# aantropov/Sailor

Measured on NVIDIA B200. Metric: Mrays/s, higher is better.
Workload: dtype f32

## Files before the change

### sailor_b200/csrc/backend.cu

```cuda
#include "backend.h"
#include "../../include/sailor_pt.h"
#include <chrono>
#include <stdio.h>
#include <array>
#include <mutex>
#include <unordered_map>
#include <thread>
#include <condition_variable>
#include <atomic>
#include <vector>

namespace spt
{
	bool Ctx::Fail(const char* what, int code)
	{
		if (ok)
		{
			ok = false;
			char buf[512];
#if !defined(SPT_EMU)
			snprintf(buf, sizeof(buf), "%s -> %s (%d)", what, cudaGetErrorString((cudaError_t)code), code);
#else
			snprintf(buf, sizeof(buf), "%s -> %d", what, code);
#endif
			error = buf;
		}
		return false;
	}

#if !defined(SPT_EMU)
	namespace
	{
		std::mutex g_pinnedPoolMutex;
		std::vector<uint32_t*> g_pinnedPool;
	}
	int Ctx::Init()
	{
		int count = 0;
		if (cudaGetDeviceCount(&count) != cudaSuccess || count <= 0)
		{
			cudaGetLastError();
			ok = false;
			error = "no CUDA device: the sailor_b200 product library has no CPU path";
			return SAILOR_PT_ERR_NO_DEVICE;
		}
		if (cudaStreamCreateWithFlags(&stream, cudaStreamNonBlocking) != cudaSuccess ||
			cudaEventCreate(&evA) != cudaSuccess || cudaEventCreate(&evB) != cudaSuccess)
		{
			Fail("cudaStreamCreate/cudaEventCreate", (int)cudaGetLastError());
			return SAILOR_PT_ERR_CUDA;
		}
		ok = true;
		return SAILOR_PT_OK;
	}
	void Ctx::Destroy()
	{
		if (pinned)
		{
			std::lock_guard<std::mutex> lock(g_pinnedPoolMutex);
			if (g_pinnedPool.size() < 64) g_pinnedPool.push_back(pinned); else cudaFreeHost(pinned);
			pinned = nullptr;
		}
		if (evA) cudaEventDestroy(evA);
		if (evB) cudaEventDestroy(evB);
		for (int i = 0; i < kMarkers; i++) { if (ev[i]) cudaEventDestroy(ev[i]); ev[i] = nullptr; }
		if (stream) cudaStreamDestroy(stream);
		evA = evB = nullptr; stream = nullptr;
	}
	void Ctx::Sync() { if (ok) SPT_CUDA_CHECK(*this, cudaStreamSynchronize(stream)); }
	void Ctx::TimerStart() { if (ok) SPT_CUDA_CHECK(*this, cudaEventRecord(evA, stream)); }
	double Ctx::TimerStop()
	{
		if (!ok) return 0.0;
		SPT_CUDA_CHECK(*this, cudaEventRecord(evB, stream));
		SPT_CUDA_CHECK(*this, cudaEventSynchronize(evB));
		float ms = 0.0f;
		if (ok) SPT_CUDA_CHECK(*this, cudaEventElapsedTime(&ms, evA, evB));
		return (double)ms * 1e-3;
	}

	void Ctx::Mark(int i)
	{
		if (!ok) return;
		if (!ev[i]) SPT_CUDA_CHECK(*this, cudaEventCreate(&ev[i]));
		if (ok) SPT_CUDA_CHECK(*this, cudaEventRecord(ev[i], stream));
	}
	void Ctx::WaitMark(int i) { if (ok) SPT_CUDA_CHECK(*this, cudaEventSynchronize(ev[i])); }
	uint32_t* Ctx::Pinned()
	{
		if (!pinned && ok)
		{
			{
				std::lock_guard<std::mutex> lock(g_pinnedPoolMutex);
				if (!g_pinnedPool.empty()) { pinned = g_pinnedPool.back(); g_pinnedPool.pop_back(); }
			}
			if (!pinned) { void* p = nullptr; SPT_CUDA_CHECK(*this, cudaHostAlloc(&p, 256 * sizeof(uint32_t), cudaHostAllocPortable)); pinned = (uint32_t*)p; }
		}
		return pinned;
	}
	void Ctx::ReadAsync(uint32_t* pinnedDst, const void* src, size_t bytes)
	{
		d2hBytes += bytes;
		if (ok) SPT_CUDA_CHECK(*this, cudaMemcpyAsync(pinnedDst, src, bytes, cudaMemcpyDeviceToHost, stream));
	}
	double Ctx::Between(int i, int j)
	{
		float ms = 0.0f;
		if (ok) SPT_CUDA_CHECK(*this, cudaEventElapsedTime(&ms, ev[i], ev[j]));
		return (double)ms * 1e-3;
	}

	namespace
	{
		std::mutex g_allocMutex;
		std::unordered_map<void*, cudaStream_t> g_allocStream;
		uint64_t g_poolReady = 0;

		void EnsurePool()
		{
			int dev = 0; cudaMemPool_t pool = nullptr;
			if (cudaGetDevice(&dev) != cudaSuccess) { cudaGetLastError(); return; }
			if (dev < 64 && (g_poolReady >> dev & 1u)) return;
			if (cudaDeviceGetDefaultMemPool(&pool, dev) == cudaSuccess)
			{
				uint64_t threshold = UINT64_MAX;
				cudaMemPoolSetAttribute(pool, cudaMemPoolAttrReleaseThreshold, &threshold);
			}
			cudaGetLastError();
			if (dev < 64) g_poolReady |= 1ull << dev;
		}
	}

	void* DevAllocBytes(Ctx& ctx, size_t bytes)
	{
		void* p = nullptr;
		if (!ctx.ok) return nullptr;
		std::lock_guard<std::mutex> lock(g_allocMutex);
		EnsurePool();
		SPT_CUDA_CHECK(ctx, cudaMallocAsync(&p, bytes, ctx.stream));
		if (!ctx.ok) return nullptr;
		g_allocStream[p] = ctx.stream;
		return p;
	}
	int DevCurrent() { int d = 0; if (cudaGetDevice(&d) != cudaSuccess) { cudaGetLastError(); d = 0; } return d; }
	int DevCount() { int n = 0; if (cudaGetDeviceCount(&n) != cudaSuccess) { cudaGetLastError(); n = 0; } return n; }
	bool DevSetCurrent(int device) { if (cudaSetDevice(device) != cudaSuccess) { cudaGetLastError(); return false; } return true; }
	void DevCopyPeer(Ctx& ctx, void* dst, int dstDevice, const void* src, int srcDevice, size_t bytes)
	{
		if (!ctx.ok || !bytes) return;
		if (dstDevice == srcDevice) SPT_CUDA_CHECK(ctx, cudaMemcpyAsync(dst, src, bytes, cudaMemcpyDeviceToDevice, ctx.stream));
// ... 249 lines not shown
			__syncthreads();
			if (warp == 0)
			{
				uint32_t w = lane < kScanThreads / 32 ? warpSums[lane] : 0;
#pragma unroll
				for (int o = 1; o < 32; o <<= 1) { const uint32_t t = __shfl_up_sync(0xffffffffu, w, o); if (lane >= o) w += t; }
				if (lane < kScanThreads / 32) warpSums[lane] = w;
			}
			__syncthreads();
			total = warpSums[kScanThreads / 32 - 1];
			const uint32_t base = warp ? warpSums[warp - 1] : 0;
			__syncthreads();
			return base + incl - v;
		}

		__global__ void __launch_bounds__(kScanThreads) k_scan_reduce(const uint32_t* __restrict__ in, uint32_t n, uint32_t* __restrict__ tileSums)
		{
			const uint32_t base = blockIdx.x * kScanTile;
			uint32_t s = 0;
#pragma unroll
			for (uint32_t k = 0; k < kScanItems; k++) { const uint32_t i = base + k * kScanThreads + threadIdx.x; if (i < n) s += in[i]; }
			uint32_t total;
			BlockExclusiveScan(s, total);
			if (threadIdx.x == 0) tileSums[blockIdx.x] = total;
		}

		__global__ void __launch_bounds__(kScanThreads) k_scan_tiles(uint32_t* tileSums, uint32_t numTiles)
		{
			uint32_t carry = 0;
			for (uint32_t base = 0; base < numTiles; base += kScanThreads)
			{
				const uint32_t i = base + threadIdx.x;
				const uint32_t v = i < numTiles ? tileSums[i] : 0;
				uint32_t total;
				const uint32_t ex = BlockExclusiveScan(v, total);
				if (i < numTiles) tileSums[i] = carry + ex;
				carry += total;
			}
			if (threadIdx.x == 0) tileSums[numTiles] = carry;
		}

		__global__ void __launch_bounds__(kScanThreads) k_scan_apply(const uint32_t* __restrict__ in, uint32_t* __restrict__ out, uint32_t n, const uint32_t* __restrict__ tileOffsets, uint32_t numTiles)
		{
			const uint32_t base = blockIdx.x * kScanTile + threadIdx.x * kScanItems;
			uint32_t v[kScanItems];
			uint32_t s = 0;
#pragma unroll
			for (uint32_t k = 0; k < kScanItems; k++) { v[k] = (base + k) < n ? in[base + k] : 0; s += v[k]; }
			uint32_t total;
			uint32_t run = tileOffsets[blockIdx.x] + BlockExclusiveScan(s, total);
#pragma unroll
			for (uint32_t k = 0; k < kScanItems; k++) { if ((base + k) < n) out[base + k] = run; run += v[k]; }
			if (blockIdx.x == 0 && threadIdx.x == 0) out[n] = tileOffsets[numTiles];
		}
	}

	void ExclusiveScanU32(Ctx& ctx, const uint32_t* in, uint32_t* out, uint32_t n, DevBuf<uint32_t>& scratch)
	{
		if (!ctx.ok) return;
		if (n == 0) { DevMemset(ctx, out, 0, sizeof(uint32_t)); return; }
		const uint32_t numTiles = (n + kScanTile - 1) / kScanTile;
		scratch.Ensure(ctx, numTiles + 1);
		if (!ctx.ok) return;
		k_scan_reduce<<<numTiles, kScanThreads, 0, ctx.stream>>>(in, n, scratch.p);
		k_scan_tiles<<<1, kScanThreads, 0, ctx.stream>>>(scratch.p, numTiles);
		k_scan_apply<<<numTiles, kScanThreads, 0, ctx.stream>>>(in, out, n, scratch.p, numTiles);
		ctx.kernelLaunches += 3;
		SPT_CUDA_CHECK(ctx, cudaGetLastError());
	}

#else
	static std::chrono::steady_clock::time_point g_t0, g_marks[64];
	static double NowS() { return std::chrono::duration<double>(std::chrono::steady_clock::now().time_since_epoch()).count(); }
	void SpanTimer::Begin(Ctx&) { t0 = NowS(); }
	void SpanTimer::End(Ctx&) { acc += NowS() - t0; used += 2; }
	double SpanTimer::Collect(Ctx&) { const double s = acc; acc = 0.0; used = 0; return s; }
	void SpanTimer::Destroy() {}
	void Ctx::Mark(int i) { g_marks[i] = std::chrono::steady_clock::now(); }
	void Ctx::WaitMark(int) {}
	uint32_t* Ctx::Pinned() { if (!pinned) pinned = (uint32_t*)calloc(256, sizeof(uint32_t)); return pinned; }
	void Ctx::ReadAsync(uint32_t* pinnedDst, const void* src, size_t bytes) { d2hBytes += bytes; memcpy(pinnedDst, src, bytes); }
	double Ctx::Between(int i, int j) { return std::chrono::duration<double>(g_marks[j] - g_marks[i]).count(); }
	int Ctx::Init() { ok = true; return SAILOR_PT_OK; }
	void Ctx::Destroy() { free(pinned); pinned = nullptr; }
	void Ctx::Sync() {}
	void Ctx::TimerStart() { g_t0 = std::chrono::steady_clock::now(); }
	double Ctx::TimerStop() { return std::chrono::duration<double>(std::chrono::steady_clock::now() - g_t0).count(); }
	void* DevAllocBytes(Ctx&, size_t bytes) { return malloc(bytes ? bytes : 1); }
	void DevFreeBytes(void* p) { free(p); }
	size_t DevMemAvailable() { return (size_t)4 << 30; }
	int DevCurrent() { return 0; }
	int DevCount() { return 1; }
	bool DevSetCurrent(int device) { return device == 0; }
	void DevCopyPeer(Ctx&, void* dst, int, const void* src, int, size_t bytes) { memcpy(dst, src, bytes); }
	void TrimDevicePool() {}
	void* DevAllocPlain(Ctx&, size_t bytes) { return malloc(bytes ? bytes : 1); }
	void DevFreePlain(void* p) { free(p); }
	void DevUpload(Ctx& ctx, void* dst, const void* src, size_t bytes) { ctx.h2dBytes += bytes; memcpy(dst, src, bytes); }
	void DevDownload(Ctx& ctx, void* dst, const void* src, size_t bytes) { ctx.d2hBytes += bytes; memcpy(dst, src, bytes); }
	int HostPin(void* p, size_t bytes) { return (p && bytes) ? 0 : -1; }
	int HostUnpin(void* p) { return p ? 0 : -1; }
	void DevMemset(Ctx&, void* dst, int byte, size_t bytes) { memset(dst, byte, bytes); }
	void DevCopy(Ctx&, void* dst, const void* src, size_t bytes) { memcpy(dst, src, bytes); }
	void ExclusiveScanU32(Ctx& ctx, const uint32_t* in, uint32_t* out, uint32_t n, DevBuf<uint32_t>&)
	{
		uint32_t s = 0;
		for (uint32_t i = 0; i < n; i++) { out[i] = s; s += in[i]; }
		out[n] = s;
		ctx.kernelLaunches += 3;
	}
#endif
}
```

### sailor_b200/csrc/backend.h

```cpp
#pragma once
#include "hd.h"
#include <stddef.h>
#include <string>
#include <vector>
#include <string.h>
#include <stdlib.h>

#if !defined(SPT_EMU)
#include <cuda_runtime.h>
#if defined(__CUDACC__)
#include <cooperative_groups.h>
#include <cooperative_groups/scan.h>
#include <cooperative_groups/reduce.h>
#endif
#endif

namespace spt
{
	struct Ctx
	{
#if !defined(SPT_EMU)
		cudaStream_t stream = nullptr;
		cudaEvent_t evA = nullptr, evB = nullptr;
		static constexpr int kMarkers = 64;
		cudaEvent_t ev[kMarkers] = {};
#endif
		uint32_t kernelLaunches = 0;
		uint64_t h2dBytes = 0, d2hBytes = 0;
		static constexpr int kMarkCall0 = 60, kMarkCall1 = 61;
		std::string error;
		bool ok = true;

		int Init();
		void Destroy();
		void Sync();
		bool Fail(const char* what, int code);
		void TimerStart();
		double TimerStop();
		void Mark(int i);
		double Between(int i, int j);
		void WaitMark(int i);
		uint32_t* pinned = nullptr;
		uint32_t* Pinned();
		void ReadAsync(uint32_t* pinnedDst, const void* src, size_t bytes);
	};

#if !defined(SPT_EMU)
#define SPT_CUDA_CHECK(ctx, call) do { cudaError_t e_ = (call); if (e_ != cudaSuccess) { (ctx).Fail(#call, (int)e_); } } while (0)
#endif

	void* DevAllocBytes(Ctx& ctx, size_t bytes);
	int DevCurrent();
	int DevCount();
	bool DevSetCurrent(int device);
	void DevCopyPeer(Ctx& ctx, void* dst, int dstDevice, const void* src, int srcDevice, size_t bytes);
	void TrimDevicePool();
	void* DevAllocPlain(Ctx& ctx, size_t bytes);
	void DevFreePlain(void* p);
	size_t DevMemAvailable();
	void DevFreeBytes(void* p);
	void DevUpload(Ctx& ctx, void* dst, const void* src, size_t bytes);
	void DevDownload(Ctx& ctx, void* dst, const void* src, size_t bytes);
	void DevMemset(Ctx& ctx, void* dst, int byte, size_t bytes);
	int HostPin(void* p, size_t bytes);
	int HostUnpin(void* p);
	void DevCopy(Ctx& ctx, void* dst, const void* src, size_t bytes);

	template<class T>
	struct DevBuf
	{
		T* p = nullptr;
		size_t n = 0;
		DevBuf() = default;
		DevBuf(const DevBuf&) = delete;
		DevBuf& operator=(const DevBuf&) = delete;
		~DevBuf() { Free(); }
		void Free() { if (p) DevFreeBytes(p); p = nullptr; n = 0; }
		void Alloc(Ctx& ctx, size_t count) { Free(); if (count) { p = (T*)DevAllocBytes(ctx, count * sizeof(T)); n = p ? count : 0; } }
		void Ensure(Ctx& ctx, size_t count) { if (count > n) Alloc(ctx, count); }
		void Upload(Ctx& ctx, const T* src, size_t count) { Ensure(ctx, count); if (count) DevUpload(ctx, p, src, count * sizeof(T)); }
		void Upload(Ctx& ctx, const std::vector<T>& v) { Upload(ctx, v.data(), v.size()); }
		void Download(Ctx& ctx, T* dst, size_t count) const { if (count) DevDownload(ctx, dst, p, count * sizeof(T)); }
		void Zero(Ctx& ctx) { if (n) DevMemset(ctx, p, 0, n * sizeof(T)); }
		void Zero(Ctx& ctx, size_t count) { if (count) DevMemset(ctx, p, 0, count * sizeof(T)); }
	};

	struct PlainBuf
	{
		unsigned char* p = nullptr; size_t n = 0;
		void Ensure(Ctx& ctx, size_t bytes)
		{
			if (bytes <= n) return;
			if (p) { ctx.Sync(); DevFreePlain(p); p = nullptr; n = 0; }
			p = (unsigned char*)DevAllocPlain(ctx, bytes); n = p ? bytes : 0;
		}
	};

#if !defined(SPT_EMU)
	__device__ __forceinline__ void atomic_min_u32(uint32_t* p, uint32_t v) { atomicMin(p, v); }
	__device__ __forceinline__ void atomic_max_u32(uint32_t* p, uint32_t v) { atomicMax(p, v); }
	__device__ __forceinline__ uint32_t atomic_add_u32(uint32_t* p, uint32_t v) { return atomicAdd(p, v); }
	__device__ __forceinline__ unsigned long long atomic_add_u64(unsigned long long* p, unsigned long long v) { return atomicAdd(p, v); }
#define SPT_KERNEL_BODY __device__ __forceinline__
#if defined(__CUDACC__)
	__device__ __forceinline__ uint32_t atomic_inc_u32_agg(uint32_t* p)
	{
		const uint32_t mask = __activemask(), lane = threadIdx.x & 31u;
		const int leader = __ffs(mask) - 1;
		uint32_t base = 0;
		if ((int)lane == leader) base = atomicAdd(p, (uint32_t)__popc(mask));
		base = __shfl_sync(mask, base, leader);
		return base + (uint32_t)__popc(mask & ((1u << lane) - 1u));
	}
	__device__ __forceinline__ uint32_t atomic_add_u32_agg(uint32_t* p, uint32_t v)
	{
		namespace cg = cooperative_groups;
		const cg::coalesced_group g = cg::coalesced_threads();
		const uint32_t excl = cg::exclusive_scan(g, v);
		const uint32_t last = g.size() - 1u;
		uint32_t base = 0;
		if (g.thread_rank() == last) base = atomicAdd(p, excl + v);
		base = g.shfl(base, last);
		return base + excl;
	}
	__device__ __forceinline__ void atomic_add_u64_agg(unsigned long long* p, unsigned long long v)
	{
		namespace cg = cooperative_groups;
// ... 92 lines not shown
```

### sailor_b200/csrc/integrator.cuh

```cuda
#pragma once
#include "pipeline.cuh"
#include "textures.cuh"
#include "lighting.cuh"
#include "blue_noise_table.h"

namespace spt
{
	struct alignas(16) PrimaryHitRec { uint32_t pixel, sample, pad0, pad1; float t, u, v; uint32_t tri; };
	static_assert(sizeof(PrimaryHitRec) == 32, "PrimaryHitRec layout");

	struct RenderStats { uint64_t rays, primarySamples, fanOutSamples, replayedRays; double secondsTraverse, secondsShade, secondsStage[4]; uint32_t traverseLaunches, batches; };

	constexpr uint32_t kNone = 0xFFFFFFFFu;
#ifndef SPT_FAN_OUT_MIN
#define SPT_FAN_OUT_MIN 8
#endif
	constexpr uint32_t kFanOutMinSamples = SPT_FAN_OUT_MIN;

	enum : uint32_t
	{
		kNfOpposite = 1u, kNfThick = 2u, kNfAlpha = 4u, kNfFirst = 8u, kNfAmbientOn = 16u,
		kNfDone = 32u,
		kNfTail = 64u,
		kNfLevel0 = 128u,
	};

	struct alignas(16) NodeRec
	{
		V3 rayO; float envIor;
		V3 rayD; uint32_t pad0;
		float t, u, v; uint32_t tri;
		float inAcc; uint32_t pNum; uint64_t rngKey;
		uint32_t bounces, flags, auxBase; float alpha;
		uint32_t parent, parentAux, nA, nS;
		V3 emissive; uint32_t child;
		V3 result; uint32_t pad1;
	};
	SPT_HD uint32_t PackNum(uint32_t samples, uint32_t ambient) { return (samples & 0xFFFFu) | (ambient << 16); }
	static_assert(sizeof(NodeRec) == 128, "NodeRec layout");

	enum : uint32_t
	{
		kRkInactive = 0, kRkLight = 1, kRkHemi = 2, kRkSample = 3, kRkOwn = 4, kRkMask = 7u,
		kRsTransRay = 16u,
		kRsHit = 64u,
		kRsSky2 = 256u,
		kRsSkipped = 512u,
	};

	struct alignas(16) RayAux
	{
		float a0, a1, a2, a3;
		float b0, b1, b2;
		uint32_t tag;
	};
	static_assert(sizeof(RayAux) == 32, "RayAux layout");

	struct alignas(16) SkyState
	{
		V3 att; uint32_t targetAux;
		V3 prev; uint32_t ignore;
		V3 start; float ior;
		V3 dir; uint32_t jAndMax;
	};
	static_assert(sizeof(SkyState) == 64, "SkyState layout");

	struct ShadeCtx;
	struct LevelInfo { uint32_t recBegin, recEnd, rayCount, auxBase; };

	struct BatchCounters
	{
		uint32_t recAlloc;
		uint32_t auxAlloc;
		uint32_t overflow;
		uint32_t skyCount[2];
		uint32_t zero;
		uint32_t fanEntries;
		uint32_t slowCount;
		uint32_t fanThreads[2];
		unsigned long long rays;
		unsigned long long fanSamples;
		LevelInfo level[66];
	};

	struct IntegratorArgs
	{
		const V4* shade; const V4* centroid; const MaterialGpu* materials; TextureSet tex; const V4* lights; uint32_t numLights;
		const uint16_t* blueNoise;
		CameraGpu cam; uint32_t rowBegin, rowEnd, msBegin, msEnd, msaa;
		uint32_t maxBounces, numSamples, numAmbientSamples; V3 ambient; uint64_t seed;
		const PrimaryHitRec* hitQueue; uint32_t queueBegin, queueCount;
		NodeRec* recs; uint32_t recCap;
		RayAux* aux; uint32_t auxCap; uint32_t hasSky;
		RayRec* rays; Hit* hits; uint32_t rayCap;
		uint8_t* status; SlowRec* slow;
		SkyState* sky[2]; RayRec* skyRays; Hit* skyHits; uint32_t skyCap;
		ShadeCtx* fan; uint32_t fanCap; uint32_t* fanSlots[2];
		BatchCounters* c;
		float* sampleBuf;
	};

	SPT_HD uint64_t Mix64(uint64_t z)
	{
		z = (z ^ (z >> 30)) * 0xBF58476D1CE4E5B9ULL; z = (z ^ (z >> 27)) * 0x94D049BB133111EBULL; return z ^ (z >> 31);
	}
	SPT_HD uint64_t PrimaryRngKey(uint64_t seed, uint32_t pixel, uint32_t msaa, uint32_t sample)
	{
		return Mix64(seed * 0x9E3779B97F4A7C15ULL + ((uint64_t)pixel * msaa + sample) + 0x632BE59BD9B4E019ULL);
	}
	SPT_HD uint64_t ChildRngKey(uint64_t key, uint32_t slot) { return Mix64(key + 0xD1B54A32D192ED03ULL * (uint64_t)(slot + 1u)); }
	struct Rng
	{
		uint64_t key; uint32_t counter;
		SPT_KERNEL_BODY uint32_t U32()
		{
			const uint64_t h = Mix64(key + 0x9E3779B97F4A7C15ULL * (uint64_t)(++counter));
			const uint32_t b0 = (uint32_t)(h & 0xFFFF) % 255u, b1 = (uint32_t)((h >> 16) & 0xFFFF) % 255u;
			const uint32_t b2 = (uint32_t)((h >> 32) & 0xFFFF) % 255u, b3 = (uint32_t)((h >> 48) & 0xFFFF) % 255u;
			return (b3 << 24) | (b2 << 16) | (b1 << 8) | b0;
		}
		SPT_KERNEL_BODY float Float01() { return (float)U32() / 4294967296.0f * (1.0f - 0.0f) + 0.0f; }
		SPT_KERNEL_BODY uint32_t Seed681() { return U32() % 681u; }
	};

	SPT_KERNEL_BODY uint32_t MaterialOfTri(const IntegratorArgs& a, uint32_t tri) { return f2u(ld4(a.centroid + tri).w); }

	SPT_KERNEL_BODY V3 HitNormalOf(const IntegratorArgs& a, uint32_t tri, float u, float v)
	{
		const V4* S = a.shade + (size_t)tri * 9;
		const V4 n0 = ld4(S), n1 = ld4(S + 1), n2 = ld4(S + 2);
		const float w = 1.0f - u - v;
		return w * v3(n0.x, n0.y, n0.z) + u * v3(n1.x, n1.y, n1.z) + v * v3(n2.x, n2.y, n2.z);
	}

	SPT_KERNEL_BODY void WriteRay(RayRec* q, uint32_t i, V3 o, V3 d, uint32_t ignore, bool active, bool anyHit = false)
	{
		RayRec r; r.ox = o.x; r.oy = o.y; r.oz = o.z; r.ignoreTri = ignore; r.dx = d.x; r.dy = d.y; r.dz = d.z; r.tmax = active ? (anyHit ? -kFltMax : kFltMax) : -1.0f;
		q[i] = r;
	}

	SPT_KERNEL_BODY void WriteAux(const IntegratorArgs& a, uint32_t g, float a0, float a1, float a2, float a3, float b0, uint32_t tag, uint32_t owner)
	{
		RayAux x; x.a0 = a0; x.a1 = a1; x.a2 = a2; x.a3 = a3; x.b0 = b0; x.b1 = u2f(owner); x.b2 = 0.0f; x.tag = tag;
		a.aux[g] = x;
	}

	SPT_KERNEL_BODY uint32_t AllocRecord(const IntegratorArgs& a)
	{
		const uint32_t i = atomic_inc_u32_agg(&a.c->recAlloc);
		if (i >= a.recCap) { a.c->overflow = 1u; return kNone; }
		return i;
	}

	SPT_KERNEL_BODY bool SkyAdvance(const IntegratorArgs& a, SkyState& s, const Hit& hit, V3& result)
	{
		if (hit.tri == kNoHit) { result = s.att; return false; }
		const MaterialGpu& m = a.materials[MaterialOfTri(a, hit.tri)];
		const V3 hn = HitNormalOf(a, hit.tri, hit.u, hit.v);
		const bool hitOpp = dot(s.dir, hn) < 0.0f;
		if (!(m.transmission > 0.0f && m.thickness > 0.0f)) { result = v3(0.0f); return false; }
		const V3 hp = s.start + s.dir * hit.t;
		const float distance = length(hp - s.prev);
		s.prev = hp;
		const V3 wn = hitOpp ? hn : -hn;
// ... 598 lines not shown
							if (x.tag & kRsSkipped) continue;
							V3 value = v3(x.a0, x.a1, x.a2);
							if (!hitSomething[j])
							{
								value = glm_clamp(value * a.ambient, 0.0f, 10.0f);
								amb2 = amb2 + value; avgPdf += x.a3; indirect = indirect + value;
							}
							else if (x.tag & kRsHit)
							{
								indirect = indirect + value;
								if (x.tag & kRsSky2) { amb2 = amb2 + value * v3(x.b0, x.b1, x.b2); avgPdf += x.a3; }
							}
							else if (bouncesLeft)
								indirect = indirect + glm_clamp(value * v3(0.0f), 0.0f, 10.0f);
							cnt += 1.0f;
						}
						g += (nS - i0 < kGatherBlock) ? nS - i0 : kGatherBlock;
					}
					amb2 = amb2 / cnt; avgPdf = avgPdf / cnt;
					const V3 ambient = amb1 + amb2;
					if (ambient.x + ambient.y + ambient.z > 0.0f)
					{
						res = res + (amb1 * PowerHeuristic((int32_t)nA, pdfHemisphere, (int32_t)cnt, avgPdf) +
							amb2 * PowerHeuristic((int32_t)cnt, avgPdf, (int32_t)nA, pdfHemisphere));
					}
					if (cnt > 0.0f) res = res + (indirect / cnt);
				}
				res = res + rec->emissive;
				if ((rec->bounces & 0xFFFFu) > 0 && (flags & kNfAlpha))
				{
					const float al = rec->alpha;
					const V3 cr = rec->child != kNone ? a.recs[rec->child].result : v3(0.0f);
					res = res * al + cr * (1.0f - al);
				}
			}
			rec->result = res;
			if (flags & kNfLevel0)
			{
				const uint32_t pixel = rec->parent, sample = rec->parentAux;
				const uint32_t x = pixel % a.cam.width, y = pixel / a.cam.width;
				const size_t idx = ((size_t)(y - a.rowBegin) * a.cam.width + x) * (a.msEnd - a.msBegin) + (sample - a.msBegin);
				a.sampleBuf[idx * 3] = res.x; a.sampleBuf[idx * 3 + 1] = res.y; a.sampleBuf[idx * 3 + 2] = res.z;
			}
			else if (rec->parentAux != kNone)
			{
				RayAux* px = a.aux + rec->parentAux;
				const V3 value = glm_clamp(v3(px->a0, px->a1, px->a2) * res, 0.0f, 10.0f);
				px->a0 = value.x; px->a1 = value.y; px->a2 = value.z;
			}
		}
	};

	struct BeginBatchKernel
	{
		BatchCounters* c; uint32_t count;
		SPT_KERNEL_BODY void operator()(uint32_t) const
		{
			c->recAlloc = count; c->auxAlloc = 0; c->overflow = 0; c->skyCount[0] = c->skyCount[1] = 0; c->zero = 0; c->fanEntries = 0; c->fanThreads[0] = c->fanThreads[1] = 0; c->slowCount = 0; c->rays = 0; c->fanSamples = 0;
			c->level[0].recBegin = 0; c->level[0].recEnd = count; c->level[0].rayCount = 0; c->level[0].auxBase = 0;
		}
	};
	struct NextLevelKernel
	{
		BatchCounters* c; uint32_t level; uint32_t recCap;
		SPT_KERNEL_BODY void operator()(uint32_t) const
		{
			const LevelInfo cur = c->level[level];
			LevelInfo nx; nx.recBegin = cur.recEnd; nx.recEnd = c->recAlloc < recCap ? c->recAlloc : recCap; nx.rayCount = 0; nx.auxBase = cur.auxBase + cur.rayCount;
			c->level[level + 1] = nx;
			c->auxAlloc = nx.auxBase;
			c->rays += cur.rayCount;
			c->fanEntries = 0; c->fanThreads[0] = c->fanThreads[1] = 0; c->slowCount = 0;
		}
	};
	struct OverflowGuardKernel
	{
		BatchCounters* c; uint32_t level;
		SPT_KERNEL_BODY void operator()(uint32_t) const
		{
			if (!c->overflow) return;
			c->level[level].rayCount = 0; c->slowCount = 0; c->skyCount[0] = c->skyCount[1] = 0;
		}
	};
	struct SkySwapKernel
	{
		BatchCounters* c; uint32_t q;
		SPT_KERNEL_BODY void operator()(uint32_t) const { c->rays += c->skyCount[q]; c->skyCount[q] = 0; }
	};

	struct ResolveKernel
	{
		const float* sampleBuf; float* image; uint32_t width, height, rowBegin, rowEnd, numSamples, msaa;
		float* running; uint32_t runningValid;
		SPT_KERNEL_BODY void operator()(uint32_t i) const
		{
			const uint32_t x = i % width, yb = i / width, y = rowBegin + yb;
			V3 acc = v3(0.0f);
			if (running && runningValid) acc = v3(running[(size_t)i * 3], running[(size_t)i * 3 + 1], running[(size_t)i * 3 + 2]);
			const float* s = sampleBuf + (size_t)i * numSamples * 3;
			for (uint32_t k = 0; k < numSamples; k++) acc = acc + v3(s[k * 3], s[k * 3 + 1], s[k * 3 + 2]);
			if (running) { running[(size_t)i * 3] = acc.x; running[(size_t)i * 3 + 1] = acc.y; running[(size_t)i * 3 + 2] = acc.z; }
			const V3 res = acc / (float)msaa;
			const size_t o = ((size_t)(height - y - 1) * width + x) * 3;
			image[o] = res.x; image[o + 1] = res.y; image[o + 2] = res.z;
		}
	};
}
```

### sailor_b200/csrc/render.cuh

```cuda
#pragma once
#include "integrator.cuh"
#include <mutex>
#include <unordered_map>

#ifndef SPT_EXPAND_MIN_BLOCKS
#define SPT_EXPAND_MIN_BLOCKS 2
#endif
#ifndef SPT_FAN_MIN_BLOCKS
#define SPT_FAN_MIN_BLOCKS 4
#endif
#ifndef SPT_CLASSIFY_MIN_BLOCKS
#define SPT_CLASSIFY_MIN_BLOCKS 1
#endif
#ifndef SPT_GATHER_MIN_BLOCKS
#define SPT_GATHER_MIN_BLOCKS 1
#endif

namespace spt
{
	struct PrimaryArgs
	{
		BvhView bvh; CameraGpu cam;
		uint32_t rowBegin, rowEnd, msBegin, msEnd, msaa; uint64_t seed; V3 ambient;
		float* sampleBuf; PrimaryHitRec* queue; uint32_t* hitCount; uint32_t total;
// ... 246 lines not shown
		bool resolved = false;
		DevDownload(ctx, &hitCount, hitCounter, 4);
		rs.rays = realSamples; rs.primarySamples = realSamples;

		if (hitCount && ctx.ok)
		{
			const uint32_t numLights = (uint32_t)D.Host().lights.size();
			const bool ambientOn = pa.ambient.x + pa.ambient.y + pa.ambient.z > 0.0f;
			const bool hasSky = ambientOn && SceneHasThickTransmission(D.Host());
			const uint32_t levels = p.maxBounces + 1u;
			uint32_t shrink = 0;
			uint32_t done = 0;
			uint64_t held = 0;
			for (const int k : { 0, 1, 2, 3, 8, 9, 10, 11, 12, 13, 14, 15 }) held += renderMem[k].n;
			const uint64_t budget = BatchBudget(held);
			if (hostTrace) fprintf(stderr, "[sailor_pt] t=%.3f ms primary pass done: %u first hits\n", (HostNow() - tFrame0) * 1e3, hitCount);
			while (done < hitCount && ctx.ok)
			{
				BatchPlan plan = PlanBatch(budget, hitCount - done, numLights, p.numAmbientSamples, p.numSamples, p.maxBounces, ambientOn, shrink);
				if (shrink == 0u && plan.firstHits > 1024u && getenv("SAILOR_PT_TEST_OVERFLOW")) { plan.auxCap = plan.auxCap / 8u + 64u; plan.recCap = plan.recCap / 8u + 64u; }
				IntegratorArgs a;
				a.shade = D.shade.p; a.centroid = D.centroid.p; a.materials = D.materials.p; a.tex.texels = D.texels.p; a.tex.textures = D.textures.p; a.tex.srgbLut = D.srgbLut.p; a.tex.texelsF = D.texelsF.p;
				a.lights = D.lights.p; a.numLights = numLights; a.blueNoise = blue;
				a.cam = cam; a.rowBegin = rowBegin; a.rowEnd = rowEnd; a.msBegin = msBegin; a.msEnd = msEnd; a.msaa = p.msaa;
				a.maxBounces = p.maxBounces; a.numSamples = p.numSamples; a.numAmbientSamples = p.numAmbientSamples;
				a.ambient = pa.ambient; a.seed = p.seed;
				a.hitQueue = queue; a.queueBegin = done; a.queueCount = plan.firstHits;
				a.recs = EnsureBytes<NodeRec>(ctx, renderMem[0], plan.recCap); a.recCap = plan.recCap;
				a.aux = EnsureBytes<RayAux>(ctx, renderMem[1], plan.auxCap); a.auxCap = plan.auxCap; a.hasSky = hasSky ? 1u : 0u;
				a.rays = EnsureBytes<RayRec>(ctx, renderMem[2], plan.rayCap); a.slow = EnsureBytes<SlowRec>(ctx, renderMem[13], plan.rayCap); a.rayCap = plan.rayCap;
				a.hits = reinterpret_cast<Hit*>(a.slow);
				a.skyCap = hasSky ? plan.skyCap : 16u;
				a.sky[0] = EnsureBytes<SkyState>(ctx, renderMem[9], (size_t)a.skyCap * 2); a.sky[1] = a.sky[0] + a.skyCap;
				a.skyRays = EnsureBytes<RayRec>(ctx, renderMem[10], (size_t)a.skyCap * 2); a.skyHits = EnsureBytes<Hit>(ctx, renderMem[11], a.skyCap);
				a.status = EnsureBytes<uint8_t>(ctx, renderMem[12], plan.auxCap);
				a.fanCap = plan.firstHits + 1024u < (1u << 24) ? plan.firstHits + 1024u : (1u << 24);
				a.fan = EnsureBytes<ShadeCtx>(ctx, renderMem[8], a.fanCap);
				a.fanSlots[0] = EnsureBytes<uint32_t>(ctx, renderMem[14], (size_t)a.fanCap * 8u); a.fanSlots[1] = a.fanSlots[0] + (size_t)a.fanCap * 4u;
				const uint32_t replayCap = plan.rayCap > a.skyCap ? plan.rayCap : a.skyCap;
				uint32_t* replayList = (useWide || useFast) ? EnsureBytes<uint32_t>(ctx, renderMem[15], replayCap) : nullptr;
				const ReplayBuffers wb = D.Replay(replayList, replayCap);
				a.c = counters; a.sampleBuf = sampleBuf;
				if (!ctx.ok) return SAILOR_PT_ERR_CUDA;
				if (hostTrace) fprintf(stderr, "[sailor_pt] t=%.3f ms batch: first hits %u of %u (done %u), budget %.1f GiB, rayCap %u auxCap %u recCap %u shrink %u\n",
					(HostNow() - tFrame0) * 1e3, plan.firstHits, hitCount, done, (double)budget / (1 << 30), plan.rayCap, plan.auxCap, plan.recCap, shrink);

				launch_for(ctx, 1, BeginBatchKernel{ counters, plan.firstHits });
				uint32_t usedLevels = levels;
				uint32_t* pin = ctx.Pinned();
				constexpr int kMarkLevel = 10;
				if (!ctx.ok || !pin) return SAILOR_PT_ERR_CUDA;
				for (uint32_t level = 0; level < levels; level++)
				{
					const LevelInfo* L = &counters->level[level];
					const uint32_t maxRecs = level == 0 ? plan.firstHits : plan.recCap;
					st[0].Begin(ctx);
					launch_for_range<SPT_EXPAND_MIN_BLOCKS>(ctx, &L->recBegin, &L->recEnd, plan.recCap, maxRecs, ExpandKernel{ a, level });
					st[0].End(ctx);
					st[1].Begin(ctx);
					launch_for_range<SPT_FAN_MIN_BLOCKS>(ctx, &counters->zero, &counters->fanThreads[0], a.fanCap * 32u, a.fanCap * 32u, FanOutKernel{ a, level, 0u });
					launch_for_range<SPT_FAN_MIN_BLOCKS>(ctx, &counters->zero, &counters->fanThreads[1], a.fanCap * 32u, a.fanCap * 32u, FanOutKernel{ a, level, 1u });
					st[1].End(ctx);
					launch_for(ctx, 1, OverflowGuardKernel{ counters, level });
					if (probeTraversal && level == 0u)
					{
						probeTraversal = false;
						const uint32_t probeN = plan.rayCap < (64u << 20) ? plan.rayCap : (64u << 20);
						double best[2] = { 1e30, 1e30 };
						for (int round = 0; round < 1 && ctx.ok; round++)
						{
							ctx.TimerStart(); LaunchTraceRaysFast(ctx, fast, view, wb, a.rays, a.hits, probeN, &L->rayCount); const double tf = ctx.TimerStop();
							ctx.TimerStart(); LaunchTraceRays(ctx, view, a.rays, a.hits, probeN, D.counter.p, &L->rayCount); const double te = ctx.TimerStop();
							if (tf < best[0]) best[0] = tf;
							if (te < best[1]) best[1] = te;
						}
						DevMemset(ctx, D.counter.p + 15, 0, sizeof(uint32_t));
						D.probeMs[0] = (float)(best[0] * 1e3); D.probeMs[1] = (float)(best[1] * 1e3);
						D.traceChoice = best[1] < best[0] * 0.97 ? 2u : 1u;
						D.Host().traversalChoice = D.traceChoice;
						useFast = D.traceChoice == 1u;
						if (hostTrace) fprintf(stderr, "[sailor_pt] traversal probe: origin-local %.3f ms, exact %.3f ms -> %s\n", best[0] * 1e3, best[1] * 1e3, useFast ? "origin-local" : "exact");
					}
					tt.Begin(ctx);
					if (useFast) LaunchTraceLevelFast(ctx, fast, view, wb, a.rays, a.hits, plan.rayCap, &L->rayCount, WavefrontOut{ a.status, &L->auxBase, a.slow, &counters->slowCount });
					else if (useWide) LaunchTraceLevelWide(ctx, wide, view, wb, a.rays, a.hits, plan.rayCap, &L->rayCount, WavefrontOut{ a.status, &L->auxBase, a.slow, &counters->slowCount });
					else LaunchTraceLevel(ctx, view, a.rays, a.hits, plan.rayCap, D.counter.p, &L->rayCount, WavefrontOut{ a.status, &L->auxBase, a.slow, &counters->slowCount });
					tt.End(ctx);
					st[2].Begin(ctx);
					launch_for_range<SPT_CLASSIFY_MIN_BLOCKS>(ctx, &counters->zero, &counters->slowCount, plan.rayCap, plan.rayCap, ClassifyKernel{ a, level });
					st[2].End(ctx);
					if (hasSky)
					{
						uint32_t q = 0;
						for (uint32_t it = 0; it < p.maxBounces; it++, q ^= 1u)
						{
							tt.Begin(ctx);
							if (useFast) LaunchTraceRaysFast(ctx, fast, view, wb, a.skyRays + (q ? a.skyCap : 0u), a.skyHits, a.skyCap, &counters->skyCount[q]);
							else if (useWide) LaunchTraceRaysWide(ctx, wide, view, wb, a.skyRays + (q ? a.skyCap : 0u), a.skyHits, a.skyCap, &counters->skyCount[q]);
							else LaunchTraceRays(ctx, view, a.skyRays + (q ? a.skyCap : 0u), a.skyHits, a.skyCap, D.counter.p, &counters->skyCount[q]);
							tt.End(ctx);
							st[2].Begin(ctx);
							launch_for_range(ctx, &counters->zero, &counters->skyCount[q], a.skyCap, a.skyCap, SkyKernel{ a, q });
							launch_for(ctx, 1, SkySwapKernel{ counters, q });
							st[2].End(ctx);
						}
					}
					launch_for(ctx, 1, NextLevelKernel{ counters, level, plan.recCap });
					if (level + 1u < levels)
					{
						ctx.ReadAsync(pin + 2u * (level + 1u), &counters->level[level + 1u].recBegin, 2u * sizeof(uint32_t));
						ctx.Mark(kMarkLevel + (int)((level + 1u) & 1u));
					}
					if (level >= 1u)
					{
						ctx.WaitMark(kMarkLevel + (int)(level & 1u));
						if (!ctx.ok) break;
						const uint32_t nAct = pin[2u * level + 1u] > pin[2u * level] ? pin[2u * level + 1u] - pin[2u * level] : 0u;
						if (hostTrace) fprintf(stderr, "[sailor_pt] t=%.3f ms   level %u was queued with %u activations\n", (HostNow() - tFrame0) * 1e3, level, nAct);
						if (!nAct) { usedLevels = level; break; }
					}
				}
				st[3].Begin(ctx);
				for (uint32_t level = usedLevels; level-- > 0;)
				{
					const LevelInfo* L = &counters->level[level];
					launch_for_range<SPT_GATHER_MIN_BLOCKS>(ctx, &L->recBegin, &L->recEnd, plan.recCap, level == 0 ? plan.firstHits : plan.recCap, GatherKernel{ a });
				}
				st[3].End(ctx);
				const bool lastBatch = (uint64_t)done + plan.firstHits >= hitCount && !prog.running;
				if (lastBatch) launch_for(ctx, rows * cam.width, ResolveKernel{ sampleBuf, dImage, cam.width, cam.height, rowBegin, rowEnd, ns, prog.norm ? prog.norm : p.msaa, prog.running, prog.runningValid ? 1u : 0u });
				struct { uint32_t recAlloc, auxAlloc, overflow, sky0, sky1, zero, fanEntries, slowCount, fan0, fan1; unsigned long long rays, fanSamples; } head;
				DevDownload(ctx, &head, counters, sizeof(head));
				if (!ctx.ok) break;
				if (hostTrace) fprintf(stderr, "[sailor_pt] t=%.3f ms   batch done (%u levels)\n", (HostNow() - tFrame0) * 1e3, usedLevels);
				if (head.overflow)
				{
					if (plan.firstHits <= 1024u || shrink > 16u) { ctx.error = "wavefront arenas overflow even for the smallest batch"; return SAILOR_PT_ERR_LIMIT; }
					shrink++;
					continue;
				}
				rs.rays += head.rays; rs.fanOutSamples += head.fanSamples; rs.batches++;
				done += plan.firstHits;
				resolved = lastBatch;
			}
		}
		if (!resolved) launch_for(ctx, rows * cam.width, ResolveKernel{ sampleBuf, dImage, cam.width, cam.height, rowBegin, rowEnd, ns, prog.norm ? prog.norm : p.msaa, prog.running, prog.runningValid ? 1u : 0u });
		ctx.Mark(1);
		ctx.Sync();
		rs.traverseLaunches = tt.Spans();
		{ uint32_t rep = 0; DevDownload(ctx, &rep, D.counter.p + 15, 4); rs.replayedRays = rep; }
		rs.secondsTraverse = tt.Collect(ctx);
		for (int k = 0; k < 4; k++) rs.secondsStage[k] = st[k].Collect(ctx);
		rs.secondsShade = ctx.Between(0, 1) - rs.secondsTraverse;
		return ctx.ok ? SAILOR_PT_OK : SAILOR_PT_ERR_CUDA;
	}
}
```

### sailor_b200/csrc/trace_fast.cuh

```cuda
#pragma once
#include "trace_kernels.cuh"
#include "wide_bvh.cuh"

namespace spt
{
	constexpr uint32_t kUpDone = 0xFFFFFFFFu;
	constexpr uint32_t kFastNone = 0xFFFFFFFFu;
	constexpr uint32_t kFastClimb = 0xFFFFFFFEu;
	constexpr uint32_t kTriLastBit = 0x80000000u;

	struct alignas(32) FHalf { float lox, loy, loz, hix, hiy, hiz; uint32_t ref, up; };
	struct alignas(64) FNode { FHalf h[2]; };
	struct alignas(64) FTri { float v0x, v0y, v0z, e1x, e1y, e1z, e2x, e2y, e2z; uint32_t id; float blox, bloy, bloz, bhix, bhiy, bhiz; };
	struct alignas(32) FStart { uint32_t up, slot; float reach[3]; uint32_t pad[3]; };
	struct FHeader { float originLimit; float pad; uint32_t r0, r1; };
	static_assert(sizeof(FNode) == 64 && sizeof(FTri) == 64 && sizeof(FStart) == 32, "fast traversal layout");

	struct FastView { const FNode* nodes; const FTri* tris; const FStart* start; const FHeader* header; const FNode* climb; uint32_t numNodes, numTris; };

	constexpr float kFastPad = 1.0f / 262144.0f;
	constexpr float kFastOriginScale = 8.0f;
#ifndef SPT_FAST_REACH_L0
#define SPT_FAST_REACH_L0 4u
#define SPT_FAST_REACH_L1 8u
// ... 556 lines not shown
	__device__ __forceinline__ uint32_t ReplaySpread(uint32_t& n) { const uint32_t shift = n <= kReplaySpreadMax ? kReplaySpreadShift : 0u; n <<= shift; return shift; }
	template<class Inner>
	struct ReplaySource
	{
		const uint32_t* list; Inner inner; uint32_t shift;
		__device__ __forceinline__ bool Load(uint32_t i, V3& o, V3& d, uint32_t& ignore, float& maxLen, bool& anyHit) const
		{
			if (i & ((1u << shift) - 1u)) return false;
			return inner.Load(list[i >> shift], o, d, ignore, maxLen, anyHit);
		}
	};
	template<class Inner>
	struct ReplaySink
	{
		const uint32_t* list; Inner inner; uint32_t shift;
		__device__ __forceinline__ void Retire(bool finished, uint32_t i, const Hit& h, bool anyHit, V3 o, V3 d) const { inner.Retire(finished, finished ? list[i >> shift] : 0u, h, anyHit, o, d); }
	};

	__global__ void __launch_bounds__(kFastBlock, SPT_FAST_MIN_BLOCKS) k_trace_fast_rays(FastView w, const RayRec* __restrict__ rays, Hit* __restrict__ hits,
		uint32_t n, const uint32_t* __restrict__ nPtr, uint32_t* __restrict__ counter, ReplayOut replay)
	{
		__shared__ uint32_t stackMem[kFastSmemWords];
		if (nPtr) { const uint32_t m = *nPtr; if (m < n) n = m; }
		QueueSource src{ rays }; QueueSink sink{ hits };
		TraceFastLoop<0>(w, n, counter, stackMem, replay, src, sink);
	}
	__global__ void __launch_bounds__(kFastBlock, SPT_FAST_MIN_BLOCKS) k_trace_fast_level(FastView w, const RayRec* __restrict__ rays, Hit* __restrict__ hits,
		uint32_t n, const uint32_t* __restrict__ nPtr, uint32_t* __restrict__ counter, WavefrontOut out, ReplayOut replay)
	{
		__shared__ uint32_t stackMem[kFastSmemWords];
		{ const uint32_t m = *nPtr; if (m < n) n = m; }
		QueueSource src{ rays }; WavefrontSink sink{ out.status + *out.auxBase, out.slow, out.slowCount };
		TraceFastLoop<SPT_FAST_EXP_MODE>(w, n, counter, stackMem, replay, src, sink);
	}
	__global__ void __launch_bounds__(kTraceBlock) k_replay_rays(BvhView bvh, const RayRec* __restrict__ rays, Hit* __restrict__ hits,
		const uint32_t* __restrict__ list, const uint32_t* __restrict__ nPtr, uint32_t cap, uint32_t* __restrict__ counter)
	{
		__shared__ uint32_t stackMem[kSmemStack * kTraceBlock];
		uint32_t n = *nPtr; if (n > cap) n = cap;
		if (!n) return;
		const uint32_t shift = ReplaySpread(n);
		ReplaySource<QueueSource> src{ list, QueueSource{ rays }, shift }; ReplaySink<QueueSink> sink{ list, QueueSink{ hits }, shift };
		TraceWarpLoop(bvh, n, counter, stackMem, src, sink);
	}
	__global__ void __launch_bounds__(kTraceBlock) k_replay_level(BvhView bvh, const RayRec* __restrict__ rays, Hit* __restrict__ hits,
		const uint32_t* __restrict__ list, const uint32_t* __restrict__ nPtr, uint32_t cap, uint32_t* __restrict__ counter, WavefrontOut out)
	{
		__shared__ uint32_t stackMem[kSmemStack * kTraceBlock];
		uint32_t n = *nPtr; if (n > cap) n = cap;
		if (!n) return;
		const uint32_t shift = ReplaySpread(n);
		ReplaySource<QueueSource> src{ list, QueueSource{ rays }, shift };
		ReplaySink<WavefrontSink> sink{ list, WavefrontSink{ out.status + *out.auxBase, out.slow, out.slowCount }, shift };
		TraceWarpLoop(bvh, n, counter, stackMem, src, sink);
	}

	inline int FastGridSize()
	{
		static int grid = 0;
		if (!grid)
		{
			int dev = 0, sms = 148, perSm = 1;
			cudaGetDevice(&dev);
			cudaDeviceGetAttribute(&sms, cudaDevAttrMultiProcessorCount, dev);
			cudaOccupancyMaxActiveBlocksPerMultiprocessor(&perSm, k_trace_fast_level, kFastBlock, 0);
			grid = sms * (perSm > 0 ? perSm : 1);
		}
		return grid;
	}
	inline int ReplayGridSize() { const int g = TraceGridSize(); return g < 296 ? g : 296; }

	struct AccumulateReplayKernel { uint32_t* c; SPT_KERNEL_BODY void operator()(uint32_t) const { c[3] += c[1]; } };

	inline void LaunchTraceRaysFast(Ctx& ctx, const FastView& w, const BvhView& bvh, const ReplayBuffers& b, const RayRec* rays, Hit* hits, uint32_t n, const uint32_t* nPtr = nullptr)
	{
		if (!n || !ctx.ok) return;
		DevMemset(ctx, b.counters, 0, 3 * sizeof(uint32_t));
		k_trace_fast_rays<<<FastGridSize(), kFastBlock, 0, ctx.stream>>>(w, rays, hits, n, nPtr, b.counters, ReplayOut{ b.replayList, b.counters + 1 });
		k_replay_rays<<<ReplayGridSize(), kTraceBlock, 0, ctx.stream>>>(bvh, rays, hits, b.replayList, b.counters + 1, b.replayCap, b.counters + 2);
		launch_for(ctx, 1, AccumulateReplayKernel{ b.counters });
		ctx.kernelLaunches += 2;
		SPT_CUDA_CHECK(ctx, cudaGetLastError());
	}
	inline void LaunchTraceLevelFast(Ctx& ctx, const FastView& w, const BvhView& bvh, const ReplayBuffers& b, const RayRec* rays, Hit* hits, uint32_t cap, const uint32_t* nPtr, const WavefrontOut& out)
	{
		if (!cap || !ctx.ok) return;
		DevMemset(ctx, b.counters, 0, 3 * sizeof(uint32_t));
		k_trace_fast_level<<<FastGridSize(), kFastBlock, 0, ctx.stream>>>(w, rays, hits, cap, nPtr, b.counters, out, ReplayOut{ b.replayList, b.counters + 1 });
		k_replay_level<<<ReplayGridSize(), kTraceBlock, 0, ctx.stream>>>(bvh, rays, hits, b.replayList, b.counters + 1, b.replayCap, b.counters + 2, out);
		launch_for(ctx, 1, AccumulateReplayKernel{ b.counters });
		ctx.kernelLaunches += 2;
		SPT_CUDA_CHECK(ctx, cudaGetLastError());
	}
#else
	inline void LaunchTraceRaysFast(Ctx& ctx, const FastView& w, const BvhView& bvh, const ReplayBuffers& b, const RayRec* rays, Hit* hits, uint32_t n, const uint32_t* nPtr = nullptr)
	{
		LocalStack st;
		if (nPtr && *nPtr < n) n = *nPtr;
		for (uint32_t i = 0; i < n; i++)
		{
			if (rays[i].tmax == -1.0f) continue;
			const V3 o = v3(rays[i].ox, rays[i].oy, rays[i].oz), d = v3(rays[i].dx, rays[i].dy, rays[i].dz);
			if (!TraceFast(w, o, d, rays[i].ignoreTri, rays[i].tmax < 0.0f, hits[i]))
			{
				TraceClosest(bvh, o, d, rays[i].ignoreTri, fabsf(rays[i].tmax), st, hits[i]);
				b.counters[3]++;
			}
		}
		ctx.kernelLaunches += 3;
	}
	inline void LaunchTraceLevelFast(Ctx& ctx, const FastView& w, const BvhView& bvh, const ReplayBuffers& b, const RayRec* rays, Hit* hits, uint32_t cap, const uint32_t* nPtr, const WavefrontOut& out)
	{
		LocalStack st;
		const uint32_t n = *nPtr < cap ? *nPtr : cap;
		for (uint32_t i = 0; i < n; i++)
		{
			if (rays[i].tmax == -1.0f) continue;
			const V3 o = v3(rays[i].ox, rays[i].oy, rays[i].oz), d = v3(rays[i].dx, rays[i].dy, rays[i].dz);
			Hit h;
			if (!TraceFast(w, o, d, rays[i].ignoreTri, rays[i].tmax < 0.0f, h))
			{
				TraceClosest(bvh, o, d, rays[i].ignoreTri, fabsf(rays[i].tmax), st, h);
				b.counters[3]++;
			}
			out.status[*out.auxBase + i] = h.tri != kNoHit ? 1 : 0;
			if (h.tri != kNoHit && !(rays[i].tmax < 0.0f)) PushSlow(out, h, rays[i], i);
		}
		ctx.kernelLaunches += 3;
	}
#endif
}
```

Measured before the change: 2926.

## Overlap classify of fast-path hits with replay kernel on a side stream

Splits the fast level trace into a walk launch and a replay launch, snapshots the slow-queue count after the walk, and runs the classify kernel for those entries on a forked side stream while the replay kernel runs on the main stream. After joining, the main classify handles only the entries the replay appended. The aim is to hide classify work behind the replay tail. It adds stream and event fork/join overhead and an extra snapshot kernel, and it relies on classify not reading hits the replay is still writing.

```diff
diff --git a/sailor_b200/csrc/backend.cu b/sailor_b200/csrc/backend.cu
--- a/sailor_b200/csrc/backend.cu
+++ b/sailor_b200/csrc/backend.cu
@@ -64,8 +64,30 @@
 		if (evA) cudaEventDestroy(evA);
 		if (evB) cudaEventDestroy(evB);
 		for (int i = 0; i < kMarkers; i++) { if (ev[i]) cudaEventDestroy(ev[i]); ev[i] = nullptr; }
+		if (evFork) cudaEventDestroy(evFork);
+		if (evJoin) cudaEventDestroy(evJoin);
+		if (side) cudaStreamDestroy(side);
 		if (stream) cudaStreamDestroy(stream);
-		evA = evB = nullptr; stream = nullptr;
+		evA = evB = evFork = evJoin = nullptr; stream = side = nullptr;
+	}
+	void Ctx::Fork()
+	{
+		if (!ok) return;
+		if (!side)
+		{
+			SPT_CUDA_CHECK(*this, cudaStreamCreateWithFlags(&side, cudaStreamNonBlocking));
+			if (ok) SPT_CUDA_CHECK(*this, cudaEventCreateWithFlags(&evFork, cudaEventDisableTiming));
+			if (ok) SPT_CUDA_CHECK(*this, cudaEventCreateWithFlags(&evJoin, cudaEventDisableTiming));
+			if (!ok) return;
+		}
+		SPT_CUDA_CHECK(*this, cudaEventRecord(evFork, stream));
+		if (ok) SPT_CUDA_CHECK(*this, cudaStreamWaitEvent(side, evFork, 0));
+	}
+	void Ctx::Join()
+	{
+		if (!ok || !side) return;
+		SPT_CUDA_CHECK(*this, cudaEventRecord(evJoin, side));
+		if (ok) SPT_CUDA_CHECK(*this, cudaStreamWaitEvent(stream, evJoin, 0));
 	}
 	void Ctx::Sync() { if (ok) SPT_CUDA_CHECK(*this, cudaStreamSynchronize(stream)); }
 	void Ctx::TimerStart() { if (ok) SPT_CUDA_CHECK(*this, cudaEventRecord(evA, stream)); }
@@ -481,6 +503,8 @@
 	void Ctx::ReadAsync(uint32_t* pinnedDst, const void* src, size_t bytes) { d2hBytes += bytes; memcpy(pinnedDst, src, bytes); }
 	double Ctx::Between(int i, int j) { return std::chrono::duration<double>(g_marks[j] - g_marks[i]).count(); }
 	int Ctx::Init() { ok = true; return SAILOR_PT_OK; }
+	void Ctx::Fork() {}
+	void Ctx::Join() {}
 	void Ctx::Destroy() { free(pinned); pinned = nullptr; }
 	void Ctx::Sync() {}
 	void Ctx::TimerStart() { g_t0 = std::chrono::steady_clock::now(); }
diff --git a/sailor_b200/csrc/backend.h b/sailor_b200/csrc/backend.h
--- a/sailor_b200/csrc/backend.h
+++ b/sailor_b200/csrc/backend.h
@@ -2,6 +2,7 @@
 #include "hd.h"
 #include <stddef.h>
 #include <string>
+#include <utility>
 #include <vector>
 #include <string.h>
 #include <stdlib.h>
@@ -24,6 +25,8 @@
 		cudaEvent_t evA = nullptr, evB = nullptr;
 		static constexpr int kMarkers = 64;
 		cudaEvent_t ev[kMarkers] = {};
+		cudaStream_t side = nullptr;
+		cudaEvent_t evFork = nullptr, evJoin = nullptr;
 #endif
 		uint32_t kernelLaunches = 0;
 		uint64_t h2dBytes = 0, d2hBytes = 0;
@@ -43,6 +46,18 @@
 		uint32_t* pinned = nullptr;
 		uint32_t* Pinned();
 		void ReadAsync(uint32_t* pinnedDst, const void* src, size_t bytes);
+		void Fork();
+		void Join();
+	};
+	struct SideScope
+	{
+		Ctx& ctx;
+#if !defined(SPT_EMU)
+		explicit SideScope(Ctx& c) : ctx(c) { std::swap(ctx.stream, ctx.side); }
+		~SideScope() { std::swap(ctx.stream, ctx.side); }
+#else
+		explicit SideScope(Ctx& c) : ctx(c) {}
+#endif
 	};
 
 #if !defined(SPT_EMU)
diff --git a/sailor_b200/csrc/integrator.cuh b/sailor_b200/csrc/integrator.cuh
--- a/sailor_b200/csrc/integrator.cuh
+++ b/sailor_b200/csrc/integrator.cuh
@@ -80,6 +80,7 @@
 		uint32_t fanThreads[2];
 		unsigned long long rays;
 		unsigned long long fanSamples;
+		uint32_t slowSplit;
 		LevelInfo level[66];
 	};
 
@@ -844,6 +845,11 @@
 			c->level[level].rayCount = 0; c->slowCount = 0; c->skyCount[0] = c->skyCount[1] = 0;
 		}
 	};
+	struct SnapSlowKernel
+	{
+		BatchCounters* c;
+		SPT_KERNEL_BODY void operator()(uint32_t) const { c->slowSplit = c->slowCount; }
+	};
 	struct SkySwapKernel
 	{
 		BatchCounters* c; uint32_t q;
diff --git a/sailor_b200/csrc/render.cuh b/sailor_b200/csrc/render.cuh
--- a/sailor_b200/csrc/render.cuh
+++ b/sailor_b200/csrc/render.cuh
@@ -352,12 +352,24 @@
 						if (hostTrace) fprintf(stderr, "[sailor_pt] traversal probe: origin-local %.3f ms, exact %.3f ms -> %s\n", best[0] * 1e3, best[1] * 1e3, useFast ? "origin-local" : "exact");
 					}
 					tt.Begin(ctx);
-					if (useFast) LaunchTraceLevelFast(ctx, fast, view, wb, a.rays, a.hits, plan.rayCap, &L->rayCount, WavefrontOut{ a.status, &L->auxBase, a.slow, &counters->slowCount });
+					if (useFast)
+					{
+						const WavefrontOut out{ a.status, &L->auxBase, a.slow, &counters->slowCount };
+						LaunchTraceLevelFastWalk(ctx, fast, view, wb, a.rays, a.hits, plan.rayCap, &L->rayCount, out);
+						launch_for(ctx, 1, SnapSlowKernel{ counters });
+						ctx.Fork();
+						{
+							SideScope side(ctx);
+							launch_for_range<SPT_CLASSIFY_MIN_BLOCKS>(ctx, &counters->zero, &counters->slowSplit, plan.rayCap, plan.rayCap, ClassifyKernel{ a, level });
+						}
+						LaunchTraceLevelFastReplay(ctx, view, wb, a.rays, a.hits, plan.rayCap, out);
+					}
 					else if (useWide) LaunchTraceLevelWide(ctx, wide, view, wb, a.rays, a.hits, plan.rayCap, &L->rayCount, WavefrontOut{ a.status, &L->auxBase, a.slow, &counters->slowCount });
 					else LaunchTraceLevel(ctx, view, a.rays, a.hits, plan.rayCap, D.counter.p, &L->rayCount, WavefrontOut{ a.status, &L->auxBase, a.slow, &counters->slowCount });
 					tt.End(ctx);
+					if (useFast) ctx.Join();
 					st[2].Begin(ctx);
-					launch_for_range<SPT_CLASSIFY_MIN_BLOCKS>(ctx, &counters->zero, &counters->slowCount, plan.rayCap, plan.rayCap, ClassifyKernel{ a, level });
+					launch_for_range<SPT_CLASSIFY_MIN_BLOCKS>(ctx, useFast ? &counters->slowSplit : &counters->zero, &counters->slowCount, plan.rayCap, plan.rayCap, ClassifyKernel{ a, level });
 					st[2].End(ctx);
 					if (hasSky)
 					{
diff --git a/sailor_b200/csrc/trace_fast.cuh b/sailor_b200/csrc/trace_fast.cuh
--- a/sailor_b200/csrc/trace_fast.cuh
+++ b/sailor_b200/csrc/trace_fast.cuh
@@ -662,14 +662,20 @@
 		ctx.kernelLaunches += 2;
 		SPT_CUDA_CHECK(ctx, cudaGetLastError());
 	}
-	inline void LaunchTraceLevelFast(Ctx& ctx, const FastView& w, const BvhView& bvh, const ReplayBuffers& b, const RayRec* rays, Hit* hits, uint32_t cap, const uint32_t* nPtr, const WavefrontOut& out)
+	inline void LaunchTraceLevelFastWalk(Ctx& ctx, const FastView& w, const BvhView&, const ReplayBuffers& b, const RayRec* rays, Hit* hits, uint32_t cap, const uint32_t* nPtr, const WavefrontOut& out)
 	{
 		if (!cap || !ctx.ok) return;
 		DevMemset(ctx, b.counters, 0, 3 * sizeof(uint32_t));
 		k_trace_fast_level<<<FastGridSize(), kFastBlock, 0, ctx.stream>>>(w, rays, hits, cap, nPtr, b.counters, out, ReplayOut{ b.replayList, b.counters + 1 });
+		ctx.kernelLaunches++;
+		SPT_CUDA_CHECK(ctx, cudaGetLastError());
+	}
+	inline void LaunchTraceLevelFastReplay(Ctx& ctx, const BvhView& bvh, const ReplayBuffers& b, const RayRec* rays, Hit* hits, uint32_t cap, const WavefrontOut& out)
+	{
+		if (!cap || !ctx.ok) return;
 		k_replay_level<<<ReplayGridSize(), kTraceBlock, 0, ctx.stream>>>(bvh, rays, hits, b.replayList, b.counters + 1, b.replayCap, b.counters + 2, out);
 		launch_for(ctx, 1, AccumulateReplayKernel{ b.counters });
-		ctx.kernelLaunches += 2;
+		ctx.kernelLaunches++;
 		SPT_CUDA_CHECK(ctx, cudaGetLastError());
 	}
 #else
@@ -689,7 +695,8 @@
 		}
 		ctx.kernelLaunches += 3;
 	}
-	inline void LaunchTraceLevelFast(Ctx& ctx, const FastView& w, const BvhView& bvh, const ReplayBuffers& b, const RayRec* rays, Hit* hits, uint32_t cap, const uint32_t* nPtr, const WavefrontOut& out)
+	inline void LaunchTraceLevelFastReplay(Ctx& ctx, const BvhView&, const ReplayBuffers&, const RayRec*, Hit*, uint32_t, const WavefrontOut&) { ctx.kernelLaunches++; }
+	inline void LaunchTraceLevelFastWalk(Ctx& ctx, const FastView& w, const BvhView& bvh, const ReplayBuffers& b, const RayRec* rays, Hit* hits, uint32_t cap, const uint32_t* nPtr, const WavefrontOut& out)
 	{
 		LocalStack st;
 		const uint32_t n = *nPtr < cap ? *nPtr : cap;
@@ -706,7 +713,7 @@
 			out.status[*out.auxBase + i] = h.tri != kNoHit ? 1 : 0;
 			if (h.tri != kNoHit && !(rays[i].tmax < 0.0f)) PushSlow(out, h, rays[i], i);
 		}
-		ctx.kernelLaunches += 3;
+		ctx.kernelLaunches += 2;
 	}
 #endif
 }
```

Result: faster. 2975, median of 6 (+1.7%).
